# vocdoni/zk-franchise-proof-circuit

Measured on AMD Instinct MI355X. Metric: zkCensus proofs/sec (nLevels=160), higher is better.
Workload: dtype u256 (8 x u32 Montgomery, BN254 Fr/Fq)

## Files before the change

zk-franchise-proof-circuit_amd/csrc/zkc_f29_g1.h:

```cpp
#pragma once
#include "zkc_f29.h"
#include "zkc_curve.h"

namespace zkc {

struct Acc29 { uint32_t X[9], Y[9], ZZ[9], ZZZ[9]; };
struct Dom29 {
    static constexpr L9 D25 = f29_dominator<FqParams>(1u << 29, 1u << 25);
    static constexpr L9 D24 = f29_dominator<FqParams>(1u << 29, 1u << 24);
    static constexpr L9 D24x3 = f29_dominator<FqParams>(3u << 29, 1u << 24);
    static constexpr L9 D26x2 = f29_dominator<FqParams>(2u << 29, 1u << 26);
    static constexpr L9 D27 = f29_dominator<FqParams>(1u << 29, 1u << 27);
};
ZKC_HD void f29_enter_fq(uint32_t r[9], const uint32_t w[8]) {
    uint32_t t[9]; f29_from_fp_shl5(t, w); f29_mul<FqParams>(r, t, F29K<FqParams>::one.l);
}

ZKC_HD bool f29_madd(Acc29& acc, const uint32_t x2[9], const uint32_t y2[9], bool& same_y) {
    typedef FqParams P;
    uint32_t Pn[9], Rn[9], nX[9], nY[9];
#pragma unroll
    for (int k = 0; k < 9; k++) { nX[k] = Dom29::D25.l[k] - acc.X[k]; nY[k] = Dom29::D25.l[k] - acc.Y[k]; }
    f29_mul_addhi<P>(Pn, x2, acc.ZZ, nX); f29_mul_addhi<P>(Rn, y2, acc.ZZZ, nY);
    if (f29_is_zero_mod_p<P>(Pn)) { same_y = f29_is_zero_mod_p<P>(Rn); return false; }
    uint32_t PP[9], PPP[9], Q[9], W[9], T[9], V[9];
    f29_sqr<P>(PP, Pn); f29_mul<P>(PPP, Pn, PP); f29_mul<P>(Q, acc.X, PP);
#pragma unroll
    for (int k = 0; k < 9; k++) T[k] = Dom29::D24x3.l[k] - PPP[k] - 2 * Q[k];
    f29_sqr_addhi<P>(acc.X, Rn, T);
    f29_sub(W, Q, acc.X, Dom29::D25);
    f29_mul2sum<P>(acc.Y, Rn, W, nY, PPP);
    f29_mul<P>(T, acc.ZZ, PP); f29_mul<P>(V, acc.ZZZ, PPP);
#pragma unroll
    for (int k = 0; k < 9; k++) { acc.ZZ[k] = T[k]; acc.ZZZ[k] = V[k]; }
    return true;
}

ZKC_HD bool f29_pt_is_inf(const Acc29& a) { uint32_t o = 0;
// ... 73 lines not shown
```

zk-franchise-proof-circuit_amd/csrc/zkc_generic.hip:

```cpp
#include <cstring>
#include <string>
#include <vector>
#include <map>
#include "zkc_prover.h"

using namespace zkc;

namespace {
Fr root_of_unity(int logn) {
    uint32_t e[8]; for (int i = 0; i < 8; i++) e[i] = FrParams::p[i]; e[0] -= 1;
    for (int i = 0; i < 8; i++) e[i] = (e[i] >> 28) | (i < 7 ? e[i + 1] << 4 : 0);
    Fr g = fp_from_u32<FrParams>(5), w = Fr::one();
    for (int i = 255; i >= 0; i--) { w = w * w; if ((e[i >> 5] >> (i & 31)) & 1) w = w * g; }
    for (int i = 28; i > logn; i--) w = w * w;
    return w;
}

__global__ void __launch_bounds__(256) zkc_fill_fr(Fr* __restrict__ dst, Fr v, uint32_t n) {
    const uint32_t i = blockIdx.x * blockDim.x + threadIdx.x;
    if (i < n) dst[i] = v;
}
__global__ void __launch_bounds__(256) zkc_g1_std_to_mont(const uint32_t* __restrict__ in, G1Affine* __restrict__ out, uint32_t n, uint32_t* __restrict__ bad) {
    const uint32_t i = blockIdx.x * blockDim.x + threadIdx.x;
    if (i >= n) return;
// ... 69 lines not shown
    ZKC_LOCK(ctx);
    ZKC_HIP_CHECK(ctx, hipSetDevice(ctx->device));
    uint32_t x[8], y[8]; memcpy(x, base_std, 32); memcpy(y, base_std + 32, 32);
    if (!fp_std_lt_p<FqParams>(x) || !fp_std_lt_p<FqParams>(y)) return zkc_fail(ctx, ZKC_ERR_BAD_ARG, "zkc_g1_mul_batch_dev: base coordinate >= q");
    G1Affine p; p.x = fp_from_std<FqParams>(x); p.y = fp_from_std<FqParams>(y);
    G1XYZZ* d_tmp = nullptr;
    ZKC_HIP_CHECK(ctx, hipMalloc((void**)&d_tmp, (size_t)n * sizeof(G1XYZZ)));
    hipLaunchKernelGGL(zkc_g1_mul_same_base, dim3((n + 63) / 64), dim3(64), 0, ctx->stream, p, (const uint32_t*)d_scalars, n, d_tmp);
    hipLaunchKernelGGL(zkc_g1_xyzz_to_std, dim3((n + 63) / 64), dim3(64), 0, ctx->stream, d_tmp, (uint32_t*)d_out, n);
    hipError_t e = hipGetLastError();
    if (e == hipSuccess) e = hipStreamSynchronize(ctx->stream);
    (void)hipFree(d_tmp);
    if (e != hipSuccess) return zkc_fail(ctx, ZKC_ERR_HIP, std::string("zkc_g1_mul_batch_dev: ") + hipGetErrorString(e));
    return ZKC_OK;
}

extern "C" int zkc_msm_g1_load_dev(zkc_ctx* ctx, const void* d_bases_std, uint32_t n, zkc_msm** out) {
    if (!ctx || !d_bases_std || !out || n == 0 || n > (1u << 21)) return zkc_fail(ctx, ZKC_ERR_BAD_ARG, "zkc_msm_g1_load_dev: bad argument (1 <= n <= 2^21)");
    ZKC_LOCK(ctx);
    ZKC_HIP_CHECK(ctx, hipSetDevice(ctx->device));
    zkc_msm* m = new zkc_msm(); m->zk.ctx = ctx; m->n = n; m->c = msm_c_for(n);
    const int nw = msm_nw(m->c);
    uint32_t* d_bad = nullptr; uint32_t bad = 0; int rc = ZKC_OK;
    auto bail = [&](int code) { if (d_bad) (void)hipFree(d_bad); if (m->zk.d_g1) (void)hipFree(m->zk.d_g1); if (m->d_red) (void)hipFree(m->d_red); m->zk.d_g1 = nullptr; msm_work_free(m->w); delete m; return code; };
    if (hipMalloc((void**)&m->zk.d_g1, (size_t)nw * n * sizeof(G1Affine)) != hipSuccess || hipMalloc((void**)&m->d_red, (size_t)n * 32) != hipSuccess ||
        hipMalloc((void**)&d_bad, 4) != hipSuccess || hipMemset(d_bad, 0, 4) != hipSuccess)
        return bail(zkc_fail(ctx, ZKC_ERR_HIP, "zkc_msm_g1_load_dev: hipMalloc failed"));
    hipLaunchKernelGGL(zkc_g1_std_to_mont, dim3((n + 255) / 256), dim3(256), 0, ctx->stream, (const uint32_t*)d_bases_std, m->zk.d_g1, n, d_bad);
    if (hipMemcpyAsync(&bad, d_bad, 4, hipMemcpyDeviceToHost, ctx->stream) != hipSuccess || hipStreamSynchronize(ctx->stream) != hipSuccess)
        return bail(zkc_fail(ctx, ZKC_ERR_HIP, "zkc_msm_g1_load_dev: base conversion failed"));
    if (bad) return bail(zkc_fail(ctx, ZKC_ERR_FORMAT, bad & 1 ? "zkc_msm_g1_load_dev: base coordinate >= q" : "zkc_msm_g1_load_dev: base not on the curve"));
    if ((rc = msm_precompute_g1(ctx, n, m->zk.d_g1, m->c))) return bail(rc);
    if ((rc = msm_work_alloc(ctx, m->w, (size_t)nw * n, (size_t)msm_half(m->c), 1, false))) return bail(rc);
    if (hipStreamSynchronize(ctx->stream) != hipSuccess) return bail(zkc_fail(ctx, ZKC_ERR_HIP, "zkc_msm_g1_load_dev: table build failed"));
    (void)hipFree(d_bad);
    *out = m;
    return ZKC_OK;
}
extern "C" int zkc_msm_g1_dev(zkc_msm* m, const void* d_scalars, uint8_t out[64]) {
    if (!m || !d_scalars || !out) return ZKC_ERR_BAD_ARG;
    zkc_ctx* ctx = m->zk.ctx;
    ZKC_LOCK(ctx);
    ZKC_HIP_CHECK(ctx, hipSetDevice(ctx->device));
    hipLaunchKernelGGL(zkc_reduce_scalars, dim3((m->n + 255) / 256), dim3(256), 0, ctx->stream, (const uint32_t*)d_scalars, m->d_red, m->n);
    ZKC_HIP_CHECK(ctx, hipGetLastError());
    m->jl.clear(); m->jl.add(m->d_red, nullptr, m->n, 0, m->n, 0, m->c);
    int rc = msm_pass_g1(&m->zk, m->w, m->jl, 0, true, ctx->stream); if (rc) return rc;
    ZKC_HIP_CHECK(ctx, hipStreamSynchronize(ctx->stream));
    const G1Affine a = xyzz_to_affine(*(const G1XYZZ*)m->w.h_results);
    uint32_t s[8]; fp_to_std<FqParams>(s, a.x); memcpy(out, s, 32); fp_to_std<FqParams>(s, a.y); memcpy(out + 32, s, 32);
    return ZKC_OK;
}
extern "C" void zkc_msm_g1_free(zkc_msm* m) {
    if (!m) return;
    ZKC_LOCK(m->zk.ctx);
    (void)hipSetDevice(m->zk.ctx->device); (void)hipStreamSynchronize(m->zk.ctx->stream);
    if (m->zk.d_g1) (void)hipFree(m->zk.d_g1);
    if (m->d_red) (void)hipFree(m->d_red);
    m->zk.d_g1 = nullptr; msm_work_free(m->w);
    delete m;
}
```

zk-franchise-proof-circuit_amd/csrc/zkc_msm.hip:

```cpp
#include <cstdio>
#include <cstddef>
#include <ctime>
#include <cstdlib>
#include <cstring>
#include <string.h>
#include <vector>
#include "zkc_prover.h"
#include "zkc_f29.h"
#include "zkc_f29_g1.h"
#include "zkc_f29_g2.h"

namespace zkc {

template <class F> struct PointIO;
template <class PP> struct PointIO<Fp<PP>> {
    typedef Fp<PP> Fq;
    static __device__ __forceinline__ Affine<Fq> load(const Affine<Fq>* p) {
        const uint4* d = reinterpret_cast<const uint4*>(p); uint4 a = d[0], b = d[1], c = d[2], e = d[3];
        Affine<Fq> r;
        r.x.v[0] = a.x; r.x.v[1] = a.y; r.x.v[2] = a.z; r.x.v[3] = a.w; r.x.v[4] = b.x; r.x.v[5] = b.y; r.x.v[6] = b.z; r.x.v[7] = b.w;
        r.y.v[0] = c.x; r.y.v[1] = c.y; r.y.v[2] = c.z; r.y.v[3] = c.w; r.y.v[4] = e.x; r.y.v[5] = e.y; r.y.v[6] = e.z; r.y.v[7] = e.w;
        return r;
    }
};
template <class BB> struct PointIO<Fq2T<BB>> {
    typedef Fq2T<BB> Fq2; typedef BB Fq;
    static __device__ __forceinline__ Affine<Fq2> load(const Affine<Fq2>* p) {
        const Affine<Fq>* q = reinterpret_cast<const Affine<Fq>*>(p);
        Affine<Fq> lo = PointIO<Fq>::load(q), hi = PointIO<Fq>::load(q + 1);
        return {{lo.x, lo.y}, {hi.x, hi.y}};
    }
};

__device__ __forceinline__ void msm_seg_range(uint32_t L, uint32_t k, uint32_t i, uint32_t& lo, uint32_t& hi) {
    lo = (uint32_t)(((uint64_t)i * L) / k); hi = (uint32_t)(((uint64_t)(i + 1) * L) / k);
}

template <int MINW>
__global__ void __launch_bounds__(128, MINW)
zkc_msm_accumulate29(const Affine<Fq>* __restrict__ table_all, const MsmJobList* __restrict__ jlp, const uint32_t* __restrict__ vals, const uint32_t* __restrict__ off,
                     const uint32_t* __restrict__ bcnt, const uint32_t* __restrict__ segoff, const uint32_t* __restrict__ seg2bucket, const uint32_t* __restrict__ perm, uint32_t nbuckets,
                     XYZZ<Fq>* __restrict__ partial, uint32_t max_segments) {
    const uint32_t gid = blockIdx.x * blockDim.x + threadIdx.x;
    uint32_t nseg = segoff[nbuckets]; if (nseg > max_segments) nseg = max_segments;
    if (gid >= nseg) return;
    const uint32_t s = perm[gid];
    const uint32_t b = seg2bucket[s];
    uint32_t lo, hi; msm_seg_range(bcnt[b], segoff[b + 1] - segoff[b], s - segoff[b], lo, hi);
    const uint32_t start = off[b] + lo, end = off[b] + hi;
    uint32_t bd, bj; jlp->decode(b, bd, bj);
    const Affine<Fq>* __restrict__ table = table_all + jlp->job[bj].tbl_off;
    constexpr uint32_t rowmask = 0x7fffffffu;
    Acc29 acc; bool inf = true;
    uint32_t v = vals[start];
    Affine<Fq> p = PointIO<Fq>::load(table + (v & rowmask));
    for (uint32_t j = start; j < end; j++) {
        const uint32_t vn = (j + 1 < end) ? vals[j + 1] : v;
        Affine<Fq> pn = PointIO<Fq>::load(table + (vn & rowmask));
        if (!p.is_inf()) {
            if (v >> 31) p.y = fp_neg(p.y);
            uint32_t x2[9], y2[9];
            f29_from_fp_shl5(x2, p.x.v); f29_from_fp_shl5(y2, p.y.v);
            bool same_y = false;
            if (inf) {
                f29_mul<FqParams>(acc.X, x2, F29K<FqParams>::one.l); f29_mul<FqParams>(acc.Y, y2, F29K<FqParams>::one.l);
#pragma unroll
                for (int k = 0; k < 9; k++) acc.ZZ[k] = acc.ZZZ[k] = F29K<FqParams>::one.l[k];
                inf = false;
            } else if (!f29_madd(acc, x2, y2, same_y)) {
                if (same_y) {
                    const XYZZ<Fq> d = xyzz_dbl_affine(p);
                    f29_enter_fq(acc.X, d.X.v); f29_enter_fq(acc.Y, d.Y.v); f29_enter_fq(acc.ZZ, d.ZZ.v); f29_enter_fq(acc.ZZZ, d.ZZZ.v);
                } else inf = true;
            }
        }
        v = vn; p = pn;
    }
    XYZZ<Fq> out = XYZZ<Fq>::inf();
    if (!inf) { out.X = f29_to_fp<FqParams>(acc.X); out.Y = f29_to_fp<FqParams>(acc.Y); out.ZZ = f29_to_fp<FqParams>(acc.ZZ); out.ZZZ = f29_to_fp<FqParams>(acc.ZZZ); }
    partial[s] = out;
}

constexpr int G2T29_WORDS = 60;
__global__ void __launch_bounds__(128)
zkc_g2_table29(const Affine<Fq2>* __restrict__ tbl, uint32_t* __restrict__ out, size_t count) {
    const size_t i = (size_t)blockIdx.x * blockDim.x + threadIdx.x;
    if (i >= count) return;
    const Affine<Fq2> a = PointIO<Fq2>::load(tbl + i);
    uint32_t* o = out + i * G2T29_WORDS;
    const Fq2 ny = fp_neg(a.y);
    f29_enter_fq(o, a.x.c0.v); f29_enter_fq(o + 9, a.x.c1.v); o[18] = a.is_inf() ? 1u : 0u; o[19] = 0;
    f29_enter_fq(o + 20, a.y.c0.v); f29_enter_fq(o + 29, a.y.c1.v); o[38] = o[39] = 0;
    f29_enter_fq(o + 40, ny.c0.v); f29_enter_fq(o + 49, ny.c1.v); o[58] = o[59] = 0;
}
// ... 476 lines not shown
    if (rc != ZKC_OK) msm_work_free(w);
    return rc;
}
void msm_work_free(MsmWork& w) {
    void* p[] = {w.vals, w.vals2, w.hist, w.bin_start, w.tilecnt, w.off, w.bcnt, w.segcnt, w.segoff, w.seg2bucket, w.seglen, w.perm, w.scan_blk, w.lencnt, w.heavy, w.d_jobs, w.d_windows,
                 w.partial, w.wres, w.results};
    for (void* q : p) if (q) (void)hipFree(q);
    if (w.h_results) (void)hipHostFree(w.h_results);
    if (w.d_tilejob) (void)hipFree(w.d_tilejob);
    for (int s = 0; s < 2; s++) { if (w.h_tilejob[s]) (void)hipHostFree(w.h_tilejob[s]); if (w.h_jobs[s]) (void)hipHostFree(w.h_jobs[s]); if (w.h_windows[s]) (void)hipHostFree(w.h_windows[s]); if (w.h_ev[s]) (void)hipEventDestroy(w.h_ev[s]); }
    w = MsmWork();
}

static const bool g_debug_sync = getenv("ZKC_DEBUG_SYNC") != nullptr;
#define ZKC_LAUNCH_CHECK(ctx, name)                                                                        \
    do { hipError_t _e = hipGetLastError(); if (_e != hipSuccess)                                          \
        return zkc_fail((ctx), ZKC_ERR_HIP, std::string(name ": ") + hipGetErrorString(_e));               \
        if (g_debug_sync) { timespec _t0, _t1; clock_gettime(CLOCK_MONOTONIC, &_t0);                        \
            _e = hipStreamSynchronize(st); clock_gettime(CLOCK_MONOTONIC, &_t1);                \
            fprintf(stderr, "[zkc] %-22s %8.3f ms  %s\n", name, (_t1.tv_sec - _t0.tv_sec) * 1e3 + (_t1.tv_nsec - _t0.tv_nsec) * 1e-6, \
                    hipGetErrorString(_e)); fflush(stderr); } } while (0)

template <class F>
static int msm_pass(zkc_zkey* zk, MsmWork& w, const Affine<F>* table, const MsmJobList& jl_in, int slot, bool to_host, hipStream_t st, hipEvent_t ev_sorted, hipEvent_t wait_before_acc = nullptr, hipEvent_t ev_acc = nullptr,
                    hipStream_t st_red = nullptr, hipEvent_t ev_red = nullptr) {
    zkc_ctx* ctx = zk->ctx;
    const int nj = jl_in.njobs;
    if (nj <= 0 || nj > w.max_jobs) return zkc_fail(ctx, ZKC_ERR_BAD_ARG, "msm_pass: job count");
    static thread_local MsmJobList jl;
    jl = jl_in;
    if (!jl.finish()) {
        std::string d = "msm_pass: jobs need at most two window sizes (the larger first) and tables that fit the entry word [" + std::to_string(nj) + " jobs:";
        for (int j = 0; j < nj && j < 16; j++) d += " c" + std::to_string(jl.job[j].c) + "/" + std::to_string(jl.job[j].count) + "/" + std::to_string(jl.job[j].tbl_count);
        return zkc_fail(ctx, ZKC_ERR_BAD_ARG, d + "]");
    }
    const size_t total = jl.total_entries;
    const uint32_t nb = jl.total_buckets;
    if (total > w.max_entries || nb > w.max_buckets) return zkc_fail(ctx, ZKC_ERR_BAD_ARG, "msm_pass: too many entries for the work space");
    const uint32_t seg = (uint32_t)std::min<size_t>(MSM_SEG, std::max<size_t>(MSM_SEG_MIN, total / 131072));
    constexpr bool kG2 = sizeof(F) == sizeof(Fq2);
    static const bool bw_off = [] { const char* e = getenv("ZKC_G2_BUCKET_WAVE"); return e && atoi(e) == 0; }();
    const uint32_t bw_slices = (uint32_t)std::min<size_t>(32, w.max_segments / std::max<uint32_t>(nb, 1u));
    const uint32_t* const g2_table29 = (kG2 && jl.job[0].c == (uint32_t)MSM_C_G2_LONE) ? zk->d_g2_29_lone : (kG2 && zk->c_deep && jl.job[0].c == (uint32_t)zk->c_deep) ? zk->d_g2_29_deep : zk->d_g2_29;
    const bool bucket_wave = kG2 && !bw_off && nb <= 8192 && bw_slices >= 1;
    uint64_t alg_bytes = 0; uint32_t maxcount = 0;
    uint64_t streamed_bytes = 0;
    for (int j = 0; j < nj; j++) {
        alg_bytes += (uint64_t)jl.job[j].tbl_count * (sizeof(Affine<F>) + 32);
        streamed_bytes += (uint64_t)jl.job[j].count * (sizeof(Affine<F>) + 32);
        maxcount = std::max(maxcount, jl.job[j].count);
    }
// ... 34 lines not shown
    }
    {
        zkc_prof_scope _ps(ctx, kG2 ? ZKC_PROF_MSM_ACC_G2 : ZKC_PROF_MSM_ACC_G1, alg_bytes, st);
        if (!kG2 && ((ctx->prof.mask >> ZKC_PROF_MSM_ACC_G1) & 1)) ctx->prof.bytes[ZKC_PROF_MSM_G1_STREAMED] += streamed_bytes;
        if constexpr (kG2) {
          if (bucket_wave) {
            ZKC_HIP_CHECK(ctx, hipMemsetAsync(w.heavy + MSM_MAX_HEAVY, 0, 4, st));
            hipLaunchKernelGGL(zkc_msm_bucketwave_g2, dim3((nb + 1) / 2, bw_slices), dim3(64), 0, st, g2_table29, (const MsmJobList*)w.d_jobs, w.vals2, w.off, w.bcnt, w.segoff, w.segcnt, w.heavy,
                               w.heavy + MSM_MAX_HEAVY, reinterpret_cast<XYZZ<Fq2>*>(partial), nb, bw_slices);
          }
          else {
            static const int g2_form = [] { const char* e = getenv("ZKC_G2_ACC"); return e ? atoi(e) : 0; }();
            if (g2_form == 2)
                hipLaunchKernelGGL(HIP_KERNEL_NAME(zkc_msm_accumulate29_g2_dma<2>), dim3((unsigned)((seg_bound + G2DMA_T - 1) / G2DMA_T)), dim3(G2DMA_T), 0, st,
                                   g2_table29, (const MsmJobList*)w.d_jobs, w.vals2, w.off, w.bcnt, w.segoff, w.seg2bucket, w.perm, nb, reinterpret_cast<XYZZ<Fq2>*>(partial), (uint32_t)w.max_segments);
            else if (g2_form == 1)
                hipLaunchKernelGGL(HIP_KERNEL_NAME(zkc_msm_accumulate29_g2_dma<1>), dim3((unsigned)((seg_bound + G2DMA_T - 1) / G2DMA_T)), dim3(G2DMA_T), 0, st,
                                   g2_table29, (const MsmJobList*)w.d_jobs, w.vals2, w.off, w.bcnt, w.segoff, w.seg2bucket, w.perm, nb, reinterpret_cast<XYZZ<Fq2>*>(partial), (uint32_t)w.max_segments);
            else
            hipLaunchKernelGGL(HIP_KERNEL_NAME(zkc_msm_accumulate29_g2<1>), dim3((unsigned)((seg_bound + 127) / 128)), dim3(128), 0, st,
                               g2_table29, (const MsmJobList*)w.d_jobs, w.vals2, w.off, w.bcnt, w.segoff, w.seg2bucket, w.perm, nb, reinterpret_cast<XYZZ<Fq2>*>(partial), (uint32_t)w.max_segments);
          }
        } else {
            hipLaunchKernelGGL(HIP_KERNEL_NAME(zkc_msm_accumulate29<2>), dim3((unsigned)((seg_bound + 127) / 128)), dim3(128), 0, st,
                               reinterpret_cast<const Affine<Fq>*>(table), (const MsmJobList*)w.d_jobs, w.vals2, w.off, w.bcnt, w.segoff, w.seg2bucket, w.perm, nb,
                               reinterpret_cast<XYZZ<Fq>*>(partial), (uint32_t)w.max_segments);
            if (acc_chain) { ZKC_HIP_CHECK(ctx, hipEventRecord(ctx->ev_acc_chain, st)); ctx->acc_chain_armed = true; }
        }
        ZKC_LAUNCH_CHECK(ctx, "zkc_msm_accumulate");
        if (ev_acc) ZKC_HIP_CHECK(ctx, hipEventRecord(ev_acc, st));
    }
    if (st_red && st_red != st) {
        if (!ev_acc) return zkc_fail(ctx, ZKC_ERR_BAD_ARG, "msm_pass: a reduction stream needs ev_acc");
        ZKC_HIP_CHECK(ctx, hipStreamWaitEvent(st_red, ev_acc, 0));
        st = st_red;
    }
    {
        zkc_prof_scope _pr(ctx, ZKC_PROF_MSM_REDUCE, 0, st);
        if constexpr (kG2) {
            hipLaunchKernelGGL(HIP_KERNEL_NAME(zkc_msm_merge29<Merge29G2>), dim3(1024), dim3(64), 0, st, reinterpret_cast<XYZZ<Fq2>*>(partial), w.segoff, w.segcnt, w.heavy,
                               w.heavy + MSM_MAX_HEAVY, (uint32_t)w.max_segments);
        } else
            hipLaunchKernelGGL(HIP_KERNEL_NAME(zkc_msm_merge29<Merge29G1>), dim3(1024), dim3(64), 0, st, reinterpret_cast<XYZZ<Fq>*>(partial), w.segoff, w.segcnt, w.heavy,
                               w.heavy + MSM_MAX_HEAVY, (uint32_t)w.max_segments);
        ZKC_LAUNCH_CHECK(ctx, "zkc_msm_merge");
        if constexpr (kG2)
            hipLaunchKernelGGL(zkc_msm_window29_g2, dim3(jl.total_windows), dim3(64), 0, st, reinterpret_cast<const XYZZ<Fq2>*>(partial), w.segoff, w.segcnt,
                               (const MsmWindow*)w.d_windows, reinterpret_cast<XYZZ<Fq2>*>(wres), (uint32_t)w.max_segments);
        else
            hipLaunchKernelGGL(zkc_msm_window29, dim3(jl.total_windows), dim3(64), 0, st, reinterpret_cast<const XYZZ<Fq>*>(partial), w.segoff, w.segcnt,
                               (const MsmWindow*)w.d_windows, reinterpret_cast<XYZZ<Fq>*>(wres), (uint32_t)w.max_segments);
        ZKC_LAUNCH_CHECK(ctx, "zkc_msm_window");
        static_assert(msm_half(MSM_C_SMALL) / MSM_VW_MIN <= MSM_MAX_VW_PER_JOB, "G2 per-job sum: one lane per virtual window");
        if (kG2 && jl.job[0].c == (uint32_t)MSM_C_G2_LONE && !zk->d_g2_29_lone) return zkc_fail(ctx, ZKC_ERR_BAD_ARG, "msm_pass: no 8-bit-window G2 table on this key");
        for (int j = 0; j < nj; j++) if ((1u << (jl.job[j].c - 1)) / jl.job[j].vw > (uint32_t)(kG2 ? MSM_MAX_VW_PER_JOB : MSM_MAX_VW_G1)) return zkc_fail(ctx, ZKC_ERR_BAD_ARG, "msm_pass: too many virtual windows in a job for the per-job sum");
        if constexpr (kG2)
            hipLaunchKernelGGL(zkc_msm_final29_g2, dim3(nj), dim3(MSM_MAX_VW_PER_JOB), 0, st, reinterpret_cast<const XYZZ<Fq2>*>(wres), (const MsmJobList*)w.d_jobs,
                               reinterpret_cast<XYZZ<Fq2>*>(results));
        else
            hipLaunchKernelGGL(zkc_msm_final29, dim3(nj), dim3(MSM_MAX_VW_G1), 0, st, reinterpret_cast<const XYZZ<Fq>*>(wres), (const MsmJobList*)w.d_jobs, reinterpret_cast<XYZZ<Fq>*>(results));
        ZKC_LAUNCH_CHECK(ctx, "zkc_msm_final");
    }
    if (to_host) ZKC_HIP_CHECK(ctx, hipMemcpyAsync(w.h_results, results, (size_t)nj * sizeof(XYZZ<F>), hipMemcpyDeviceToHost, st));
    if (ev_red) ZKC_HIP_CHECK(ctx, hipEventRecord(ev_red, st));
    return ZKC_OK;
}
int msm_pass_g1(zkc_zkey* zk, MsmWork& w, const MsmJobList& jl, int slot, bool to_host, hipStream_t st, hipEvent_t ev_sorted, hipEvent_t ev_acc, hipStream_t st_red, hipEvent_t ev_red) {
    return msm_pass<Fq>(zk, w, zk->d_g1, jl, slot, to_host, st, ev_sorted, nullptr, ev_acc, st_red, ev_red);
}
int msm_pass_g2(zkc_zkey* zk, MsmWork& w, const MsmJobList& jl, int slot, bool to_host, hipStream_t st, hipEvent_t wait_before_acc) { return msm_pass<Fq2>(zk, w, zk->d_g2, jl, slot, to_host, st, nullptr, wait_before_acc); }

}
```

zk-franchise-proof-circuit_amd/csrc/zkc_prove.hip:

```cpp
#include "zkc_prover.h"
#include "zkc_fixedbase.h"
#include "zkc_hostparse.h"
#include "zkc_kernels.h"
#include <cstring>
#include <ctime>
#include <cstdio>
#include <algorithm>
#include <atomic>

using namespace zkc;

static void matvec_launch(zkc_zkey* zk, zkc_lane& L, const uint32_t* d_wtns0, int nb, hipStream_t mv) {
    const uint32_t n = zk->n, nv = zk->nVars;
    static const bool unit_off = [] { const char* e = getenv("ZKC_MATVEC_UNITS"); return e && atoi(e) == 0; }();
    const bool units = zk->n_unit_coeffs > 0 && nv <= 3 * (size_t)n && !unit_off;
    if (units) hipLaunchKernelGGL(zkc_wtns_mont, dim3((nv + 255) / 256, nb), dim3(256), 0, mv, (const Fr*)d_wtns0, (size_t)nv, L.d_t, 3 * (size_t)n, nv);
    hipLaunchKernelGGL(zkc_matvec_jds, dim3((2 * n + 63 * zk->nlong + 255) / 256, nb), dim3(256), 0, mv, zk->d_perm, zk->d_rowlen, zk->d_jdptr, zk->d_col, zk->d_val,
                       (const Fr*)d_wtns0, (size_t)nv, L.d_abc, (int)n, zk->nlong, units ? (const Fr*)L.d_t : (const Fr*)nullptr, 3 * (size_t)n);
    hipLaunchKernelGGL(zkc_pointwise_mul, dim3((n + 255) / 256, nb), dim3(256), 0, mv, L.d_abc, (int)n);
}
static constexpr uint32_t MATVEC_LONG = 16;

namespace {
uint32_t rd32(const uint8_t* p) { uint32_t v; memcpy(&v, p, 4); return v; }
// ... 34 lines not shown
    for (int i = threadIdx.x; i < 2 * (end - start); i += 64) { uint4 x = w[i], y = t[i]; diff |= (x.x ^ y.x) | (x.y ^ y.y) | (x.z ^ y.z) | (x.w ^ y.w); }
    const unsigned long long any = __ballot(diff != 0);
    if (threadIdx.x == 0) flags[((size_t)b * 2 + tree) * n + g] = any ? 1u : 0u;
}

extern "C" __global__ void __launch_bounds__(64)
zkc_input_depths(const uint32_t* __restrict__ inputs, int nInputs, int n, uint32_t* __restrict__ out) {
    const int b = blockIdx.x, tree = blockIdx.y;
    const uint32_t* sib = inputs + ((size_t)b * nInputs + 12 + (size_t)tree * n) * 8;
    int d = 0;
    for (int i = threadIdx.x; i < n; i += 64) {
        const uint4* q = reinterpret_cast<const uint4*>(sib + 8 * (size_t)i); const uint4 x = q[0], y = q[1];
        if (x.x | x.y | x.z | x.w | y.x | y.y | y.z | y.w) d = i + 1;
    }
    for (int m = 32; m >= 1; m >>= 1) { const int o = __shfl_xor(d, m, 64); d = o > d ? o : d; }
    if (threadIdx.x == 0) out[2 * b + tree] = (uint32_t)d;
}

extern "C" void zkc_zkey_free(zkc_zkey* zk) {
    if (!zk) return;
    ZKC_LOCK(zk->ctx);
    (void)hipSetDevice(zk->ctx->device);
    (void)hipStreamSynchronize(zk->ctx->stream);
    void* ptrs[] = {zk->d_perm, zk->d_rowlen, zk->d_jdptr, zk->d_col, zk->d_val, zk->d_tw_fwd, zk->d_tw_inv, zk->d_tw_fwd29, zk->d_tw_inv29, zk->d_coset, zk->d_coset_br, zk->d_g1, zk->d_g2, zk->d_g2_29, zk->d_g2_29_lone, zk->d_g2_29_deep,
                    zk->d_tblDelta1, zk->d_tblAlpha1, zk->d_tblBeta1, zk->d_tblDelta2, zk->d_fb4, zk->d_fb4g2, zk->d_depths};
    for (void* p : ptrs) if (p) (void)hipFree(p);
    for (auto& kv : zk->fold.vmaps) if (kv.second.d) (void)hipFree(kv.second.d);
    for (void* q : {(void*)zk->fold.d_foldA, (void*)zk->fold.d_foldB1, (void*)zk->fold.d_foldC, (void*)zk->fold.d_foldB2}) if (q) (void)hipFree(q);
    if (zk->h_depths) (void)hipHostFree(zk->h_depths);
    for (auto& c : zk->call) { for (void* q : {(void*)c.d_rs, (void*)c.d_proofs, (void*)c.d_flags, (void*)c.d_status3}) if (q) (void)hipFree(q); if (c.h_flags) (void)hipHostFree(c.h_flags); if (c.h_out) (void)hipHostFree(c.h_out); if (c.h_rs) (void)hipHostFree(c.h_rs); if (c.h_xyzz) (void)hipHostFree(c.h_xyzz); if (c.h_early) (void)hipHostFree(c.h_early); if (c.d_xyzz) (void)hipFree(c.d_xyzz); for (hipEvent_t e : c.ev_done) if (e) (void)hipEventDestroy(e); for (hipEvent_t e : c.ev_chunk) (void)hipEventDestroy(e); }
    if (zk->ctx->lanes) for (int l = 0; l < zk->nlanes; l++) for (hipStream_t q : {zk->ctx->lanes[l].st, zk->ctx->lanes[l].st2, zk->ctx->lanes[l].fin, zk->ctx->lanes[l].red}) if (q) (void)hipStreamSynchronize(q);
    delete zk;
}

static size_t dev_free_bytes() { size_t f = 0, t = 0; if (hipMemGetInfo(&f, &t) != hipSuccess) { (void)hipGetLastError(); return 0; } return f; }
static int fold_prepare(zkc_zkey* zk);
static int fb4_prepare(zkc_zkey* zk);
struct LaneNeed { size_t abc, p, fin, bs, e1, b1, e2, b2; int j1, j2; };
static LaneNeed lane_need(const zkc_zkey* zk, int inflight) {
    const uint32_t n = zk->n, nv = zk->nVars; const int NWS = msm_nw(zk->c_sec), NWB = msm_nw(zk->c_h);
    const size_t per_proof_entries = (size_t)NWS * 3 * nv + (size_t)NWB * n;
    const size_t per_proof_buckets = 3 * (size_t)msm_half(std::max(zk->c_sec, zk->c_deep)) + msm_half(zk->c_h);
    LaneNeed nd; nd.abc = 3 * (size_t)n * inflight; nd.p = 8 * (size_t)n * inflight; nd.fin = finalize_scratch_bytes(inflight); nd.bs = 2 * 2 * 8 * (size_t)nv;
    nd.e1 = per_proof_entries * inflight; nd.b1 = per_proof_buckets * inflight; nd.j1 = 4 * inflight;
    nd.e2 = (size_t)NWS * nv * inflight; nd.b2 = (size_t)msm_half(std::max(zk->c_sec, zk->c_deep)) * inflight; nd.j2 = inflight;
    return nd;
}
// ... 203 lines not shown
            if (e2 != hipSuccess) return bail(zkc_fail(ctx, ZKC_ERR_HIP, std::string("lone-proof G2 table: ") + hipGetErrorString(e2)));
        }
    }
    const char* e_inf = getenv("ZKC_INFLIGHT");
    zk->max_inflight = opt_inflight > 0 ? std::min(opt_inflight, MSM_MAX_JOBS / 4) : e_inf ? std::max(1, std::min(atoi(e_inf), MSM_MAX_JOBS / 4)) : zk->nLevels >= 0 ? 64 : 96;
    {
        const size_t per_proof_entries = (size_t)NWS * 3 * nv + (size_t)NWB * n, census_pass = 96ull * (22ull * 3 * 82754 + 15ull * 131072);
        const int fit = (int)std::max<size_t>(1, census_pass / std::max<size_t>(per_proof_entries, 1));
        zk->max_inflight = std::min(zk->max_inflight, fit);
    }
    { const char* e_l = getenv("ZKC_LANES"); zk->nlanes = opt_lanes > 0 ? std::min(opt_lanes, (int)MAX_LANES) : e_l ? std::max(1, std::min(atoi(e_l), (int)MAX_LANES)) : zk->nLevels >= 0 ? (int)MAX_LANES : 1; }
    zk->serial_streams = getenv("ZKC_SERIAL_STREAMS") != nullptr;
    if ((rc = lanes_ensure(zk, 1, 0, 1))) return bail(rc);
    {
        FixedBase<Fq> td(zk->delta1), ta(zk->alpha1), tb(zk->beta1); FixedBase<Fq2> t2(zk->delta2);
        if ((rc = dmalloc(ctx, &zk->d_tblDelta1, td.tab.size())) || (rc = dmalloc(ctx, &zk->d_tblAlpha1, ta.tab.size())) ||
            (rc = dmalloc(ctx, &zk->d_tblBeta1, tb.tab.size())) || (rc = dmalloc(ctx, &zk->d_tblDelta2, t2.tab.size()))) return bail(rc);
        ZKC_UP(zk->d_tblDelta1, td.tab.data(), td.tab.size() * sizeof(G1Affine)); ZKC_UP(zk->d_tblAlpha1, ta.tab.data(), ta.tab.size() * sizeof(G1Affine));
        ZKC_UP(zk->d_tblBeta1, tb.tab.data(), tb.tab.size() * sizeof(G1Affine)); ZKC_UP(zk->d_tblDelta2, t2.tab.data(), t2.tab.size() * sizeof(G2Affine));
    }
    ZKC_HIP_BAIL(hipStreamSynchronize(ctx->stream));
    if (zk->nLevels >= 0 && (rc = fold_prepare(zk))) return bail(rc);
    if ((rc = fb4_prepare(zk))) return bail(rc);
    { const size_t f = dev_free_bytes(), grown = ctx_work_bytes(ctx) > work_at_entry ? ctx_work_bytes(ctx) - work_at_entry : 0; zk->bytes_tables = free_at_entry > f + grown ? free_at_entry - f - grown : 0; }
    *out = zk;
    return ZKC_OK;
#undef ZKC_UP
#undef ZKC_HIP_BAIL
}

int zkc::prove_reserve(zkc_zkey* zk, int inflight) {
    if (!zk) return ZKC_ERR_BAD_ARG;
    ZKC_LOCK(zk->ctx);
    ZKC_HIP_CHECK(zk->ctx, hipSetDevice(zk->ctx->device));
    return lanes_ensure(zk, inflight);
}
extern "C" int zkc_zkey_pass_info(const zkc_zkey* zk, int* pass_size, int* lanes) {
    if (!zk) return ZKC_ERR_BAD_ARG;
    if (pass_size) *pass_size = zk->max_inflight; if (lanes) *lanes = zk->nlanes;
    return ZKC_OK;
}
extern "C" int zkc_zkey_info(const zkc_zkey* zk, uint32_t* nVars, uint32_t* nPublic, uint32_t* domainSize) {
    if (!zk) return ZKC_ERR_BAD_ARG;
    if (nVars) *nVars = zk->nVars; if (nPublic) *nPublic = zk->nPub; if (domainSize) *domainSize = zk->n;
    return ZKC_OK;
}
// ... 487 lines not shown
```

zk-franchise-proof-circuit_amd/csrc/zkc_prover.h:

```cpp
#pragma once
#include <cstring>
#include "zkc_internal.h"
#include "zkc_curve.h"

namespace zkc {
constexpr int MSM_C_BIG = 17, MSM_C_SMALL = 12;
constexpr int MSM_C_G2_LONE = 8;
inline long long first_unreduced_wire(const void* w, size_t count) {
    const uint8_t* p = (const uint8_t*)w;
    for (size_t i = 0; i < count; i++) {
        uint32_t t[8]; memcpy(t, p + 32 * i, 32);
        if (t[7] >= FrParams::p[7] && !fp_std_lt_p<FrParams>(t)) return (long long)i;
    }
    return -1;
}
inline std::string unreduced_wire_msg(long long wire) { return "Witness value at wire " + std::to_string(wire) + " is not below the field order r"; }
inline int msm_c_for(size_t W) { return W < 12000 ? 12 : W < 22000 ? 13 : W < 90000 ? 15 : W < 180000 ? 16 : 17; }
constexpr int msm_nw(int c) { return (254 + c) / c; }
constexpr int msm_half(int c) { return 1 << (c - 1); }
constexpr int MSM_VW_MIN = 64, MSM_MAX_VW_PER_JOB = 64;
constexpr int MSM_MAX_VW_G1 = 256;
constexpr int MSM_SEG_MIN = 16;
#ifndef ZKC_MSM_SEG
#define ZKC_MSM_SEG 128
#endif
constexpr int MSM_SEG = ZKC_MSM_SEG;
constexpr int MSM_MERGE_T = 8;
constexpr int MSM_MAX_HEAVY = 1 << 20;
constexpr int MSM_MAX_JOBS = 512;
constexpr int MAX_LANES = 4, CALL_SLOTS = 4;

struct MsmJob {
    const uint32_t* scalars;
    const uint32_t* vmap;
    uint32_t count;
    uint32_t tbl_off;
    uint32_t tbl_count;
    int32_t pt_shift;
    uint32_t c, nw, vw;
    uint32_t ent_off, win_off;
    uint32_t bucket0, bin0, hbits, lbits, tile0, cnt0;
};
struct FinalizeArgs {
    const G1XYZZ* r1; const G2XYZZ* r2;
    const G1XYZZ *foldA, *foldB1, *foldC; const G2XYZZ* foldB2; int fold_n;
    uint8_t dc[MSM_MAX_JOBS / 4], ds[MSM_MAX_JOBS / 4];
    const G1Affine *tblDelta1, *tblAlpha1, *tblBeta1; const G2Affine* tblDelta2;
    G1Affine alpha1; G2Affine beta2;
    const uint8_t* rs; uint8_t* out;
// ... 84 lines not shown
    hipStream_t st = nullptr, st2 = nullptr, fin = nullptr;
    hipStream_t red = nullptr; hipEvent_t ev_red = nullptr;
    zkc::Fr *d_abc = nullptr, *d_t = nullptr; uint32_t* d_p = nullptr;
    void* d_fin = nullptr;
    uint32_t* d_bs = nullptr;
    zkc::MsmWork w1, w2;
    size_t cap_abc = 0, cap_p = 0, cap_fin = 0, cap_bs = 0, bytes = 0; bool made = false;
    hipEvent_t ev_msm = nullptr, ev_msm2 = nullptr, ev_sorted = nullptr, ev_ntt = nullptr, ev_mv = nullptr, ev_acc = nullptr, ev_fin[2] = {nullptr, nullptr}; int npass = 0;
};

struct zkc_zkey {
    zkc_ctx* ctx = nullptr;
    uint32_t nVars = 0, nPub = 0, n = 0, logn = 0, nCoeffs = 0;
    int nLevels = -1;
    zkc::G1Affine alpha1, beta1, delta1;
    zkc::G2Affine beta2, gamma2, delta2;
    std::vector<zkc::G1Affine> ic;
    uint32_t *d_perm = nullptr, *d_rowlen = nullptr, *d_jdptr = nullptr, *d_col = nullptr; zkc::Fr* d_val = nullptr; uint32_t nlong = 0;
    uint32_t n_unit_coeffs = 0;
    zkc::Fr *d_tw_fwd = nullptr, *d_tw_inv = nullptr, *d_coset = nullptr;
    zkc::Fr *d_coset_br = nullptr;
    uint32_t *d_tw_fwd29 = nullptr, *d_tw_inv29 = nullptr;
    zkc::G1Affine* d_g1 = nullptr; zkc::G2Affine* d_g2 = nullptr;
    uint32_t* d_g2_29 = nullptr;
    uint32_t* d_g2_29_lone = nullptr;
    uint32_t offA = 0, offB1 = 0, offC = 0, offH = 0;
    int c_deep = 0; uint32_t offA_deep = 0, offB1_deep = 0, offC_deep = 0; uint32_t* d_g2_29_deep = nullptr;
    int c_h = zkc::MSM_C_BIG;
    int c_sec = zkc::MSM_C_SMALL;
    int max_inflight = 0;
    uint8_t sha256[32] = {0};
    size_t bytes_tables = 0;
    uint8_t fingerprint[32] = {0};
    int nlanes = 1; bool serial_streams = false;
    zkc::G1Affine *d_tblDelta1 = nullptr, *d_tblAlpha1 = nullptr, *d_tblBeta1 = nullptr; zkc::G2Affine* d_tblDelta2 = nullptr;
    uint32_t *d_depths = nullptr, *h_depths = nullptr; size_t depths_cap = 0;
    zkc::G1XYZZ* d_fb4 = nullptr; zkc::G2XYZZ* d_fb4g2 = nullptr; int fb4_bases = 0;
    struct CallSlot {
        uint8_t *d_rs = nullptr, *d_proofs = nullptr; size_t cap = 0;
        uint8_t* h_out = nullptr;
        uint8_t* h_rs = nullptr;
        uint8_t *d_xyzz = nullptr, *h_xyzz = nullptr; std::vector<uint8_t> as_xyzz;
        hipEvent_t ev_done[zkc::MAX_LANES] = {};
        std::vector<hipEvent_t> ev_chunk;
        uint32_t lanes_used = 0;
        int B = 0; bool pending = false;
// ... 19 lines not shown
int ntt_pair_run(zkc_ctx* ctx, hipStream_t st, Fr* data, const uint32_t* tw_inv29, const uint32_t* tw_fwd29, const Fr* scale_br, int logn, int nvec);
int ntt_bitrev_table(zkc_ctx* ctx, const Fr* d_src, Fr** out, int logn);
int msm_work_alloc(zkc_ctx* ctx, MsmWork& w, size_t max_entries, size_t max_buckets, int max_jobs, bool g2);
void msm_work_free(MsmWork& w);
int msm_pass_g1(zkc_zkey* zk, MsmWork& w, const MsmJobList& jl, int slot, bool to_host, hipStream_t st, hipEvent_t ev_sorted = nullptr, hipEvent_t ev_acc = nullptr,
                hipStream_t st_red = nullptr, hipEvent_t ev_red = nullptr);
int msm_pass_g2(zkc_zkey* zk, MsmWork& w, const MsmJobList& jl, int slot, bool to_host, hipStream_t st, hipEvent_t wait_before_acc = nullptr);
int msm_bucket_entries(zkc_ctx* ctx, MsmWork& w, const MsmJobList& jl, hipStream_t st, unsigned long long* d_entry_counter = nullptr);
int msm_build_segments(zkc_ctx* ctx, MsmWork& w, const MsmJobList& jl, uint32_t seg, size_t seg_bound, hipStream_t st);
int finalize_launch(zkc_ctx* ctx, hipStream_t st, const FinalizeArgs& a, int nproofs);
int finalize_tree_g2_launch(zkc_ctx* ctx, hipStream_t st, const FinalizeArgs& a, int nproofs);
int fb4_build(zkc_ctx* ctx, hipStream_t st, const G1XYZZ* d_bases, int nbases, G1XYZZ* d_out, const G2XYZZ& delta2, const G2XYZZ& beta2, const G2XYZZ& beta2_base, G2XYZZ* d_out2);
int blind_scalars_launch(zkc_ctx* ctx, hipStream_t st, const BlindArgs& a, int nproofs);
int prove_batch_begin(zkc_zkey* zk, int cs, const void* d_wtns, uint32_t nWitness, int B, const uint8_t* rs, bool want_publics, const void* d_inputs, int32_t* d_status,
                      int lane0 = -1, hipEvent_t wait_first = nullptr, const uint8_t* host_depths = nullptr, bool no_early = false);
int prove_batch_finish(zkc_zkey* zk, int cs, uint8_t* proofs, uint8_t* publics);
int prove_reserve(zkc_zkey* zk, int inflight);
int zkey_load_opts(zkc_ctx* ctx, const void* zkey_bytes, size_t len, int nlanes, int max_inflight, zkc_zkey** out);
size_t zkey_device_bytes(const zkc_zkey* zk, size_t* tables, size_t* work);
size_t finalize_scratch_bytes(int nproofs);
int msm_precompute_g1(zkc_ctx* ctx, uint32_t count, G1Affine* d_table, int c);
int msm_precompute_g2(zkc_ctx* ctx, uint32_t count, G2Affine* d_table, int c);
int msm_g2_table29(zkc_ctx* ctx, const G2Affine* d_table, uint32_t* d_out, size_t count);
int fold_group_sums_g1(zkc_ctx* ctx, const G1Affine* tbl, const uint32_t* d_scalars, const uint32_t* d_wires, uint32_t nw, int32_t pt_shift,
                       const uint32_t* d_gstart, uint32_t ngroups, G1XYZZ* h_out);
int fold_group_sums_g1_ws(zkc_ctx* ctx, const G1Affine* tbl, const uint32_t* d_scalars, const uint32_t* d_wires, uint32_t nw, const uint32_t* d_gstart, uint32_t ngroups,
                          G1XYZZ* d_tmp , G1XYZZ* d_out , G1XYZZ* h_out);
int fold_group_sums_g2(zkc_ctx* ctx, const G2Affine* tbl, const uint32_t* d_scalars, const uint32_t* d_wires, uint32_t nw, int32_t pt_shift,
                       const uint32_t* d_gstart, uint32_t ngroups, G2XYZZ* h_out);
}
```

Baseline: 3097.

## Precompute G1 MSM table in 29-bit limb Montgomery form for accumulation

Adds a one-time kernel at key load that converts the affine G1 base table into a 20-word row: both coordinates already in 29-bit limbs and the f29 Montgomery domain, plus an infinity flag. The old affine table is then freed. The accumulate kernel gathers these rows with vector loads, negates y with a dominator subtraction, and seeds the accumulator without the per-point limb conversion and the two initial multiplies. The min-waves launch bound also rises from 2 to 3. The trade-off is 80-byte rows instead of 64-byte points, so the random gather moves more bytes and needs more memory, and the tighter launch bound may cause register spills.

```diff
diff --git a/zk-franchise-proof-circuit_amd/csrc/zkc_f29_g1.h b/zk-franchise-proof-circuit_amd/csrc/zkc_f29_g1.h
--- a/zk-franchise-proof-circuit_amd/csrc/zkc_f29_g1.h
+++ b/zk-franchise-proof-circuit_amd/csrc/zkc_f29_g1.h
@@ -11,9 +11,15 @@
     static constexpr L9 D24x3 = f29_dominator<FqParams>(3u << 29, 1u << 24);
     static constexpr L9 D26x2 = f29_dominator<FqParams>(2u << 29, 1u << 26);
     static constexpr L9 D27 = f29_dominator<FqParams>(1u << 29, 1u << 27);
+    static constexpr L9 D22 = f29_dominator<FqParams>(1u << 29, 1u << 22);
 };
 ZKC_HD void f29_enter_fq(uint32_t r[9], const uint32_t w[8]) {
     uint32_t t[9]; f29_from_fp_shl5(t, w); f29_mul<FqParams>(r, t, F29K<FqParams>::one.l);
+}
+
+ZKC_HD void f29_g1_row_y(uint32_t y2[9], const uint32_t y[9], bool neg) {
+#pragma unroll
+    for (int k = 0; k < 9; k++) y2[k] = neg ? Dom29::D22.l[k] - y[k] : y[k];
 }
 
 ZKC_HD bool f29_madd(Acc29& acc, const uint32_t x2[9], const uint32_t y2[9], bool& same_y) {
diff --git a/zk-franchise-proof-circuit_amd/csrc/zkc_generic.hip b/zk-franchise-proof-circuit_amd/csrc/zkc_generic.hip
--- a/zk-franchise-proof-circuit_amd/csrc/zkc_generic.hip
+++ b/zk-franchise-proof-circuit_amd/csrc/zkc_generic.hip
@@ -115,7 +115,7 @@
     zkc_msm* m = new zkc_msm(); m->zk.ctx = ctx; m->n = n; m->c = msm_c_for(n);
     const int nw = msm_nw(m->c);
     uint32_t* d_bad = nullptr; uint32_t bad = 0; int rc = ZKC_OK;
-    auto bail = [&](int code) { if (d_bad) (void)hipFree(d_bad); if (m->zk.d_g1) (void)hipFree(m->zk.d_g1); if (m->d_red) (void)hipFree(m->d_red); m->zk.d_g1 = nullptr; msm_work_free(m->w); delete m; return code; };
+    auto bail = [&](int code) { if (d_bad) (void)hipFree(d_bad); if (m->zk.d_g1) (void)hipFree(m->zk.d_g1); if (m->zk.d_g1_29) (void)hipFree(m->zk.d_g1_29); if (m->d_red) (void)hipFree(m->d_red); m->zk.d_g1 = nullptr; m->zk.d_g1_29 = nullptr; msm_work_free(m->w); delete m; return code; };
     if (hipMalloc((void**)&m->zk.d_g1, (size_t)nw * n * sizeof(G1Affine)) != hipSuccess || hipMalloc((void**)&m->d_red, (size_t)n * 32) != hipSuccess ||
         hipMalloc((void**)&d_bad, 4) != hipSuccess || hipMemset(d_bad, 0, 4) != hipSuccess)
         return bail(zkc_fail(ctx, ZKC_ERR_HIP, "zkc_msm_g1_load_dev: hipMalloc failed"));
@@ -124,9 +124,12 @@
         return bail(zkc_fail(ctx, ZKC_ERR_HIP, "zkc_msm_g1_load_dev: base conversion failed"));
     if (bad) return bail(zkc_fail(ctx, ZKC_ERR_FORMAT, bad & 1 ? "zkc_msm_g1_load_dev: base coordinate >= q" : "zkc_msm_g1_load_dev: base not on the curve"));
     if ((rc = msm_precompute_g1(ctx, n, m->zk.d_g1, m->c))) return bail(rc);
+    if (hipMalloc((void**)&m->zk.d_g1_29, (size_t)nw * n * G1T29_WORDS * 4) != hipSuccess) return bail(zkc_fail(ctx, ZKC_ERR_HIP, "zkc_msm_g1_load_dev: hipMalloc failed"));
+    if ((rc = msm_g1_table29(ctx, m->zk.d_g1, m->zk.d_g1_29, (size_t)nw * n))) return bail(rc);
     if ((rc = msm_work_alloc(ctx, m->w, (size_t)nw * n, (size_t)msm_half(m->c), 1, false))) return bail(rc);
     if (hipStreamSynchronize(ctx->stream) != hipSuccess) return bail(zkc_fail(ctx, ZKC_ERR_HIP, "zkc_msm_g1_load_dev: table build failed"));
     (void)hipFree(d_bad);
+    (void)hipFree(m->zk.d_g1); m->zk.d_g1 = nullptr;
     *out = m;
     return ZKC_OK;
 }
@@ -148,8 +151,8 @@
     if (!m) return;
     ZKC_LOCK(m->zk.ctx);
     (void)hipSetDevice(m->zk.ctx->device); (void)hipStreamSynchronize(m->zk.ctx->stream);
-    if (m->zk.d_g1) (void)hipFree(m->zk.d_g1);
+    if (m->zk.d_g1_29) (void)hipFree(m->zk.d_g1_29);
     if (m->d_red) (void)hipFree(m->d_red);
-    m->zk.d_g1 = nullptr; msm_work_free(m->w);
+    m->zk.d_g1_29 = nullptr; msm_work_free(m->w);
     delete m;
 }
diff --git a/zk-franchise-proof-circuit_amd/csrc/zkc_msm.hip b/zk-franchise-proof-circuit_amd/csrc/zkc_msm.hip
--- a/zk-franchise-proof-circuit_amd/csrc/zkc_msm.hip
+++ b/zk-franchise-proof-circuit_amd/csrc/zkc_msm.hip
@@ -36,9 +36,34 @@
     lo = (uint32_t)(((uint64_t)i * L) / k); hi = (uint32_t)(((uint64_t)(i + 1) * L) / k);
 }
 
+__global__ void __launch_bounds__(128)
+zkc_g1_table29(const Affine<Fq>* __restrict__ tbl, uint32_t* __restrict__ out, size_t count) {
+    const size_t i = (size_t)blockIdx.x * blockDim.x + threadIdx.x;
+    if (i >= count) return;
+    const Affine<Fq> a = PointIO<Fq>::load(tbl + i);
+    uint32_t w[G1T29_WORDS];
+    f29_enter_fq(w, a.x.v); f29_enter_fq(w + 9, a.y.v); w[18] = a.is_inf() ? 1u : 0u; w[19] = 0;
+    uint4* o = reinterpret_cast<uint4*>(out + i * G1T29_WORDS);
+#pragma unroll
+    for (int k = 0; k < 5; k++) o[k] = make_uint4(w[4 * k], w[4 * k + 1], w[4 * k + 2], w[4 * k + 3]);
+}
+int msm_g1_table29(zkc_ctx* ctx, const G1Affine* d_table, uint32_t* d_out, size_t count) {
+    hipLaunchKernelGGL(zkc_g1_table29, dim3((unsigned)((count + 127) / 128)), dim3(128), 0, ctx->stream, d_table, d_out, count);
+    hipError_t e = hipGetLastError();
+    if (e != hipSuccess) return zkc_fail(ctx, ZKC_ERR_HIP, std::string("zkc_g1_table29: ") + hipGetErrorString(e));
+    return ZKC_OK;
+}
+struct G1Row { uint32_t w[G1T29_WORDS - 1]; };
+__device__ __forceinline__ G1Row g1_row_load(const uint32_t* p) {
+    const uint4* q = reinterpret_cast<const uint4*>(p); G1Row r;
+#pragma unroll
+    for (int i = 0; i < 4; i++) { const uint4 v = q[i]; r.w[4 * i] = v.x; r.w[4 * i + 1] = v.y; r.w[4 * i + 2] = v.z; r.w[4 * i + 3] = v.w; }
+    const uint3 t = *reinterpret_cast<const uint3*>(p + 16); r.w[16] = t.x; r.w[17] = t.y; r.w[18] = t.z;
+    return r;
+}
 template <int MINW>
 __global__ void __launch_bounds__(128, MINW)
-zkc_msm_accumulate29(const Affine<Fq>* __restrict__ table_all, const MsmJobList* __restrict__ jlp, const uint32_t* __restrict__ vals, const uint32_t* __restrict__ off,
+zkc_msm_accumulate29(const uint32_t* __restrict__ table29_all, const MsmJobList* __restrict__ jlp, const uint32_t* __restrict__ vals, const uint32_t* __restrict__ off,
                      const uint32_t* __restrict__ bcnt, const uint32_t* __restrict__ segoff, const uint32_t* __restrict__ seg2bucket, const uint32_t* __restrict__ perm, uint32_t nbuckets,
                      XYZZ<Fq>* __restrict__ partial, uint32_t max_segments) {
     const uint32_t gid = blockIdx.x * blockDim.x + threadIdx.x;
@@ -49,27 +74,29 @@
     uint32_t lo, hi; msm_seg_range(bcnt[b], segoff[b + 1] - segoff[b], s - segoff[b], lo, hi);
     const uint32_t start = off[b] + lo, end = off[b] + hi;
     uint32_t bd, bj; jlp->decode(b, bd, bj);
-    const Affine<Fq>* __restrict__ table = table_all + jlp->job[bj].tbl_off;
+    const uint32_t* __restrict__ table29 = table29_all + (size_t)jlp->job[bj].tbl_off * G1T29_WORDS;
     constexpr uint32_t rowmask = 0x7fffffffu;
     Acc29 acc; bool inf = true;
     uint32_t v = vals[start];
-    Affine<Fq> p = PointIO<Fq>::load(table + (v & rowmask));
+    G1Row p = g1_row_load(table29 + (size_t)(v & rowmask) * G1T29_WORDS);
     for (uint32_t j = start; j < end; j++) {
         const uint32_t vn = (j + 1 < end) ? vals[j + 1] : v;
-        Affine<Fq> pn = PointIO<Fq>::load(table + (vn & rowmask));
-        if (!p.is_inf()) {
-            if (v >> 31) p.y = fp_neg(p.y);
+        const G1Row pn = g1_row_load(table29 + (size_t)(vn & rowmask) * G1T29_WORDS);
+        if (!p.w[18]) {
             uint32_t x2[9], y2[9];
-            f29_from_fp_shl5(x2, p.x.v); f29_from_fp_shl5(y2, p.y.v);
+#pragma unroll
+            for (int k = 0; k < 9; k++) x2[k] = p.w[k];
+            f29_g1_row_y(y2, p.w + 9, (v >> 31) != 0);
             bool same_y = false;
             if (inf) {
-                f29_mul<FqParams>(acc.X, x2, F29K<FqParams>::one.l); f29_mul<FqParams>(acc.Y, y2, F29K<FqParams>::one.l);
-#pragma unroll
-                for (int k = 0; k < 9; k++) acc.ZZ[k] = acc.ZZZ[k] = F29K<FqParams>::one.l[k];
+#pragma unroll
+                for (int k = 0; k < 9; k++) { acc.X[k] = x2[k]; acc.Y[k] = y2[k]; acc.ZZ[k] = acc.ZZZ[k] = F29K<FqParams>::one.l[k]; }
+                f29_carry(acc.Y);
                 inf = false;
             } else if (!f29_madd(acc, x2, y2, same_y)) {
                 if (same_y) {
-                    const XYZZ<Fq> d = xyzz_dbl_affine(p);
+                    Affine<Fq> a; a.x = f29_to_fp<FqParams>(x2); a.y = f29_to_fp<FqParams>(y2);
+                    const XYZZ<Fq> d = xyzz_dbl_affine(a);
                     f29_enter_fq(acc.X, d.X.v); f29_enter_fq(acc.Y, d.Y.v); f29_enter_fq(acc.ZZ, d.ZZ.v); f29_enter_fq(acc.ZZZ, d.ZZZ.v);
                 } else inf = true;
             }
@@ -592,11 +619,12 @@
                     hipGetErrorString(_e)); fflush(stderr); } } while (0)
 
 template <class F>
-static int msm_pass(zkc_zkey* zk, MsmWork& w, const Affine<F>* table, const MsmJobList& jl_in, int slot, bool to_host, hipStream_t st, hipEvent_t ev_sorted, hipEvent_t wait_before_acc = nullptr, hipEvent_t ev_acc = nullptr,
+static int msm_pass(zkc_zkey* zk, MsmWork& w, const MsmJobList& jl_in, int slot, bool to_host, hipStream_t st, hipEvent_t ev_sorted, hipEvent_t wait_before_acc = nullptr, hipEvent_t ev_acc = nullptr,
                     hipStream_t st_red = nullptr, hipEvent_t ev_red = nullptr) {
     zkc_ctx* ctx = zk->ctx;
     const int nj = jl_in.njobs;
     if (nj <= 0 || nj > w.max_jobs) return zkc_fail(ctx, ZKC_ERR_BAD_ARG, "msm_pass: job count");
+    if (sizeof(F) == sizeof(Fq) && !zk->d_g1_29) return zkc_fail(ctx, ZKC_ERR_BAD_ARG, "msm_pass: no G1 table on this key");
     static thread_local MsmJobList jl;
     jl = jl_in;
     if (!jl.finish()) {
@@ -677,8 +705,8 @@
                                g2_table29, (const MsmJobList*)w.d_jobs, w.vals2, w.off, w.bcnt, w.segoff, w.seg2bucket, w.perm, nb, reinterpret_cast<XYZZ<Fq2>*>(partial), (uint32_t)w.max_segments);
           }
         } else {
-            hipLaunchKernelGGL(HIP_KERNEL_NAME(zkc_msm_accumulate29<2>), dim3((unsigned)((seg_bound + 127) / 128)), dim3(128), 0, st,
-                               reinterpret_cast<const Affine<Fq>*>(table), (const MsmJobList*)w.d_jobs, w.vals2, w.off, w.bcnt, w.segoff, w.seg2bucket, w.perm, nb,
+            hipLaunchKernelGGL(HIP_KERNEL_NAME(zkc_msm_accumulate29<3>), dim3((unsigned)((seg_bound + 127) / 128)), dim3(128), 0, st,
+                               (const uint32_t*)zk->d_g1_29, (const MsmJobList*)w.d_jobs, w.vals2, w.off, w.bcnt, w.segoff, w.seg2bucket, w.perm, nb,
                                reinterpret_cast<XYZZ<Fq>*>(partial), (uint32_t)w.max_segments);
             if (acc_chain) { ZKC_HIP_CHECK(ctx, hipEventRecord(ctx->ev_acc_chain, st)); ctx->acc_chain_armed = true; }
         }
@@ -721,8 +749,8 @@
     return ZKC_OK;
 }
 int msm_pass_g1(zkc_zkey* zk, MsmWork& w, const MsmJobList& jl, int slot, bool to_host, hipStream_t st, hipEvent_t ev_sorted, hipEvent_t ev_acc, hipStream_t st_red, hipEvent_t ev_red) {
-    return msm_pass<Fq>(zk, w, zk->d_g1, jl, slot, to_host, st, ev_sorted, nullptr, ev_acc, st_red, ev_red);
-}
-int msm_pass_g2(zkc_zkey* zk, MsmWork& w, const MsmJobList& jl, int slot, bool to_host, hipStream_t st, hipEvent_t wait_before_acc) { return msm_pass<Fq2>(zk, w, zk->d_g2, jl, slot, to_host, st, nullptr, wait_before_acc); }
-
-}
+    return msm_pass<Fq>(zk, w, jl, slot, to_host, st, ev_sorted, nullptr, ev_acc, st_red, ev_red);
+}
+int msm_pass_g2(zkc_zkey* zk, MsmWork& w, const MsmJobList& jl, int slot, bool to_host, hipStream_t st, hipEvent_t wait_before_acc) { return msm_pass<Fq2>(zk, w, jl, slot, to_host, st, nullptr, wait_before_acc); }
+
+}
diff --git a/zk-franchise-proof-circuit_amd/csrc/zkc_prove.hip b/zk-franchise-proof-circuit_amd/csrc/zkc_prove.hip
--- a/zk-franchise-proof-circuit_amd/csrc/zkc_prove.hip
+++ b/zk-franchise-proof-circuit_amd/csrc/zkc_prove.hip
@@ -80,7 +80,7 @@
     ZKC_LOCK(zk->ctx);
     (void)hipSetDevice(zk->ctx->device);
     (void)hipStreamSynchronize(zk->ctx->stream);
-    void* ptrs[] = {zk->d_perm, zk->d_rowlen, zk->d_jdptr, zk->d_col, zk->d_val, zk->d_tw_fwd, zk->d_tw_inv, zk->d_tw_fwd29, zk->d_tw_inv29, zk->d_coset, zk->d_coset_br, zk->d_g1, zk->d_g2, zk->d_g2_29, zk->d_g2_29_lone, zk->d_g2_29_deep,
+    void* ptrs[] = {zk->d_perm, zk->d_rowlen, zk->d_jdptr, zk->d_col, zk->d_val, zk->d_tw_fwd, zk->d_tw_inv, zk->d_tw_fwd29, zk->d_tw_inv29, zk->d_coset, zk->d_coset_br, zk->d_g1, zk->d_g1_29, zk->d_g2, zk->d_g2_29, zk->d_g2_29_lone, zk->d_g2_29_deep,
                     zk->d_tblDelta1, zk->d_tblAlpha1, zk->d_tblBeta1, zk->d_tblDelta2, zk->d_fb4, zk->d_fb4g2, zk->d_depths};
     for (void* p : ptrs) if (p) (void)hipFree(p);
     for (auto& kv : zk->fold.vmaps) if (kv.second.d) (void)hipFree(kv.second.d);
@@ -330,6 +330,9 @@
     ZKC_HIP_BAIL(hipStreamSynchronize(ctx->stream));
     if (zk->nLevels >= 0 && (rc = fold_prepare(zk))) return bail(rc);
     if ((rc = fb4_prepare(zk))) return bail(rc);
+    if ((rc = dmalloc(ctx, &zk->d_g1_29, (size_t)G1T29_WORDS * g1_points)) || (rc = msm_g1_table29(ctx, zk->d_g1, zk->d_g1_29, g1_points))) return bail(rc);
+    ZKC_HIP_BAIL(hipStreamSynchronize(ctx->stream));
+    ZKC_HIP_BAIL(hipFree(zk->d_g1)); zk->d_g1 = nullptr;
     { const size_t f = dev_free_bytes(), grown = ctx_work_bytes(ctx) > work_at_entry ? ctx_work_bytes(ctx) - work_at_entry : 0; zk->bytes_tables = free_at_entry > f + grown ? free_at_entry - f - grown : 0; }
     *out = zk;
     return ZKC_OK;
diff --git a/zk-franchise-proof-circuit_amd/csrc/zkc_prover.h b/zk-franchise-proof-circuit_amd/csrc/zkc_prover.h
--- a/zk-franchise-proof-circuit_amd/csrc/zkc_prover.h
+++ b/zk-franchise-proof-circuit_amd/csrc/zkc_prover.h
@@ -25,6 +25,7 @@
 #define ZKC_MSM_SEG 128
 #endif
 constexpr int MSM_SEG = ZKC_MSM_SEG;
+constexpr int G1T29_WORDS = 20;
 constexpr int MSM_MERGE_T = 8;
 constexpr int MSM_MAX_HEAVY = 1 << 20;
 constexpr int MSM_MAX_JOBS = 512;
@@ -155,6 +156,7 @@
     zkc::Fr *d_coset_br = nullptr;
     uint32_t *d_tw_fwd29 = nullptr, *d_tw_inv29 = nullptr;
     zkc::G1Affine* d_g1 = nullptr; zkc::G2Affine* d_g2 = nullptr;
+    uint32_t* d_g1_29 = nullptr;
     uint32_t* d_g2_29 = nullptr;
     uint32_t* d_g2_29_lone = nullptr;
     uint32_t offA = 0, offB1 = 0, offC = 0, offH = 0;
@@ -220,6 +222,7 @@
 int msm_precompute_g1(zkc_ctx* ctx, uint32_t count, G1Affine* d_table, int c);
 int msm_precompute_g2(zkc_ctx* ctx, uint32_t count, G2Affine* d_table, int c);
 int msm_g2_table29(zkc_ctx* ctx, const G2Affine* d_table, uint32_t* d_out, size_t count);
+int msm_g1_table29(zkc_ctx* ctx, const G1Affine* d_table, uint32_t* d_out, size_t count);
 int fold_group_sums_g1(zkc_ctx* ctx, const G1Affine* tbl, const uint32_t* d_scalars, const uint32_t* d_wires, uint32_t nw, int32_t pt_shift,
                        const uint32_t* d_gstart, uint32_t ngroups, G1XYZZ* h_out);
 int fold_group_sums_g1_ws(zkc_ctx* ctx, const G1Affine* tbl, const uint32_t* d_scalars, const uint32_t* d_wires, uint32_t nw, const uint32_t* d_gstart, uint32_t ngroups,
```

Measured after the change: 3077. About the same (-0.7%).
